# uni-medical/UniMedVL

Hardware: AMD Instinct MI355X
Metric: VQA greedy decode tokens/s, UniMedVL-14B (BAGEL-7B-MoT dims), batch 8 x 448x448 per GPU (higher is better)
Workload: dtype bf16; 1 GPU; configs[1]: UniMedVL-14B bf16 VQA greedy decode, batch=8 448x448, 1xMI355X; batch_per_gpu=8, image=448x448, parallelism=dp1, decode=hipGraph

## Files before the change

### include/unimedvl_hip.h

```cpp
#ifndef UNIMEDVL_HIP_H
#define UNIMEDVL_HIP_H
#include <stddef.h>
#include <stdint.h>

#ifdef __cplusplus
extern "C" {
#endif

typedef void* umv_stream_t;

int umv_version(void);
const char* umv_last_error(void);

size_t umv_packed_weight_elems(int N, int K);
int umv_pack_weight_bf16(const uint16_t* w, uint16_t* packed, int N, int K, umv_stream_t stream);
size_t umv_repacked_weight_elems(int N, int K, int th);
int umv_repack_weight_rows_bf16(const uint16_t* packed16, uint16_t* out, int N, int K, int th, umv_stream_t stream);
int umv_pack_weight_swiglu_bf16(const uint16_t* gate, const uint16_t* up, uint16_t* packed, int I, int K,
                                umv_stream_t stream);

enum {
    UMV_EPI_BIAS = 1,
    UMV_EPI_GELU_TANH = 2,
    UMV_EPI_SILU = 4,
    UMV_EPI_RESIDUAL = 8,
    UMV_EPI_SWIGLU = 16,
    UMV_EPI_OUT_F32 = 32
};
typedef struct {
    uint64_t seed;
    int64_t  draw;
    uint32_t stream;
    float    temperature;
    int32_t  top_k;
    float    top_p;
    float    min_p;
    float    repetition_penalty, presence_penalty, frequency_penalty;
} umv_row_sampling;
typedef struct {
    const uint16_t* x;
    int64_t ldx;
    const uint16_t* wp;
    const uint16_t* bias;
    const uint16_t* residual;
    int64_t ldr;
    void* out;
    int64_t ldo;
    const int32_t* row_idx;
    int M, N, K;
    int epilogue;
    const uint16_t* norm_w;
    float norm_eps;
    int tile_rows;
    const float* w_scale;
    int k_splits;
    int64_t split_stride;
    uint64_t* argmax_partial;
    int64_t x_rows;
    float sample_temperature;
    uint64_t sample_seed;
    const int64_t* sample_step;
    float* lse_partial;
} umv_gemm_args;
int umv_gemm_bf16(const umv_gemm_args* a, umv_stream_t stream);
int umv_gemm_bf16_rows(const umv_gemm_args* a, const umv_row_sampling* rows, umv_stream_t stream);
int umv_gemm_tile_config(int M, int N, int K);

size_t umv_packed_weight_fp8_bytes(int N, int K);
int umv_quantize_pack_weight_fp8(const uint16_t* w, const uint16_t* w_up, uint8_t* packed8, float* scale, uint16_t* deq,
                                 uint16_t* deq_up, int rows, int K, umv_stream_t stream);
int umv_gemm_fp8w(const umv_gemm_args* a, umv_stream_t stream);
int umv_gemm_fp8w_rows(const umv_gemm_args* a, const umv_row_sampling* rows, umv_stream_t stream);

size_t umv_packed_weight_mxfp4_bytes(int N, int K);
int umv_quantize_pack_weight_mxfp4(const uint16_t* w, const uint16_t* w_up, uint8_t* packed4, uint16_t* deq, uint16_t* deq_up,
                                   int rows, int K, umv_stream_t stream);
int umv_gemm_mxfp4w(const umv_gemm_args* a, umv_stream_t stream);
int umv_gemm_mxfp4t(const umv_gemm_args* a, umv_stream_t stream);

size_t umv_packed_weight_z13_bytes(int N, int K);
int umv_pack_weight_z13(const uint16_t* packed16, uint8_t* z13, int N, int K, umv_stream_t stream);
int umv_gemm_z13w(const umv_gemm_args* a, const void* z13, umv_stream_t stream);
int umv_gemm_z13w_rows(const umv_gemm_args* a, const void* z13, const umv_row_sampling* rows, umv_stream_t stream);

size_t umv_packed_weight_fp8_mfma_bytes(int N, int K);
int umv_repack_weight_fp8_mfma(const uint8_t* packed8, uint8_t* out, int N, int K, umv_stream_t stream);
int umv_quantize_act_fp8(const uint16_t* x, int64_t ldx, const int32_t* row_idx, uint8_t* xq, int64_t ldq, float* x_scale,
                         uint16_t* deq, int64_t ldd, int M, int K, umv_stream_t stream);
typedef struct {
    const uint8_t* xq;
    int64_t ldq;
    const float* x_scale;
    const uint8_t* wp;
    const float* w_scale;
    const uint16_t* bias;
    const uint16_t* residual;
    int64_t ldr;
    void* out;
    int64_t ldo;
    const int32_t* row_idx;
    int M, N, K;
    int epilogue;
} umv_gemm8_args;
int umv_gemm_fp8a8w(const umv_gemm8_args* a, umv_stream_t stream);

int umv_rmsnorm_bf16(const uint16_t* x, const uint16_t* w, const uint16_t* w_gen, const int32_t* expert,
                     uint16_t* out, int T, int H, float eps, umv_stream_t stream);
int umv_residual_rmsnorm_bf16(const float* partials, int n_splits, int64_t split_stride, int64_t ldp, uint16_t* seq,
                              const uint16_t* w, uint16_t* out, int T, int H, float eps, umv_stream_t stream);
int umv_layernorm_bf16(const uint16_t* x, const uint16_t* w, const uint16_t* b, uint16_t* out, int T, int H,
                       float eps, umv_stream_t stream);
int umv_embed_gather_bf16(const uint16_t* table, const int64_t* ids, const int32_t* out_rows, uint16_t* out,
                          int T, int H, umv_stream_t stream);
int umv_add_rows_bf16(const uint16_t* a, const uint16_t* bcast, const uint16_t* table, const int64_t* idx,
                      const int32_t* out_rows, uint16_t* out, int T, int H, umv_stream_t stream);
int umv_argmax_bf16(const uint16_t* logits, int64_t ld, int64_t* out_ids, int M, int V, umv_stream_t stream);
int umv_sample_bf16(const uint16_t* logits, int64_t ld, int64_t* out_ids, int M, int V, float temperature, uint64_t seed,
                    const int64_t* step, umv_stream_t stream);
int umv_cast_pad_f32_bf16(const float* x, int64_t ldx, uint16_t* out, int64_t ldo, int T, int K, int Kp,
                          umv_stream_t stream);
int umv_patchify_f32_bf16(const float* img, int C, int H, int W, int p, uint16_t* out, int64_t ldo, int Kp, umv_stream_t stream);


typedef struct {
    const uint16_t* qkv;
    uint16_t* q_out;
    uint16_t* k_slab;
    uint16_t* vt_slab;
    int64_t k_seg_stride, k_head_stride, v_seg_stride, v_head_stride, v_d_stride;
    const int32_t *tok_seg, *tok_slot, *tok_pos, *expert;
    const uint16_t *q_norm_w, *k_norm_w, *q_norm_w_gen, *k_norm_w_gen;
    const uint16_t *cos_tab, *sin_tab;
    int T, nq, nkv, hd;
    float eps;
    int fp32_chain;
    const float* qkv_partials;
    int n_splits;
    int64_t split_stride;
    const uint16_t* qkv_bias;
    const int32_t* page_table;
    int page_table_stride;
} umv_qkv_post_args;
int umv_qkv_post(const umv_qkv_post_args* a, umv_stream_t stream);

typedef struct {
    const uint16_t* q;
    uint16_t* out;
    const int32_t* cu_q;
    const int32_t* kv_len;
    const uint16_t* k_slab;
    const uint16_t* vt_slab;
    int64_t k_seg_stride, k_head_stride, v_seg_stride, v_head_stride, v_d_stride;
    int nseg, nq, nkv, hd, causal;
    int max_q;
    int max_kv;
    int nsplit;
    void* workspace;
    int64_t q_row_stride, k_key_stride;
    int variant;
    uint32_t* stats;
    const int32_t* page_table;
    int page_table_stride;
    int wave_split;
} umv_attn_args;
#define UMV_KV_PAGE 256
#define UMV_KV_PAGE_LOG2 8
// ... 127 lines not shown
```

### unimedvl_amd/_lib.py

```python
import ctypes as C
import os

HERE = os.path.dirname(os.path.abspath(__file__))
LIB_PATH = os.environ.get("UMV_LIB_PATH") or os.path.join(HERE, "lib", "libunimedvl_hip.so")

EPI_BIAS, EPI_GELU_TANH, EPI_SILU, EPI_RESIDUAL, EPI_SWIGLU, EPI_OUT_F32 = 1, 2, 4, 8, 16, 32


class GemmArgs(C.Structure):
    _fields_ = [
        ("x", C.c_void_p), ("ldx", C.c_int64), ("wp", C.c_void_p), ("bias", C.c_void_p),
        ("residual", C.c_void_p), ("ldr", C.c_int64), ("out", C.c_void_p), ("ldo", C.c_int64),
        ("row_idx", C.c_void_p), ("M", C.c_int), ("N", C.c_int), ("K", C.c_int), ("epilogue", C.c_int),
        ("norm_w", C.c_void_p), ("norm_eps", C.c_float), ("tile_rows", C.c_int), ("w_scale", C.c_void_p),
        ("k_splits", C.c_int), ("split_stride", C.c_int64), ("argmax_partial", C.c_void_p), ("x_rows", C.c_int64),
        ("sample_temperature", C.c_float), ("sample_seed", C.c_uint64), ("sample_step", C.c_void_p),
        ("lse_partial", C.c_void_p),
    ]


class QkvPostArgs(C.Structure):
    _fields_ = [
        ("qkv", C.c_void_p), ("q_out", C.c_void_p), ("k_slab", C.c_void_p), ("vt_slab", C.c_void_p),
        ("k_seg_stride", C.c_int64), ("k_head_stride", C.c_int64), ("v_seg_stride", C.c_int64),
# ... 16 lines not shown
        ("v_head_stride", C.c_int64), ("v_d_stride", C.c_int64),
        ("nseg", C.c_int), ("nq", C.c_int), ("nkv", C.c_int), ("hd", C.c_int), ("causal", C.c_int),
        ("max_q", C.c_int), ("max_kv", C.c_int), ("nsplit", C.c_int), ("workspace", C.c_void_p),
        ("q_row_stride", C.c_int64), ("k_key_stride", C.c_int64),
        ("variant", C.c_int), ("stats", C.c_void_p),
        ("page_table", C.c_void_p), ("page_table_stride", C.c_int), ("wave_split", C.c_int),
    ]


ATTN_FORCE, ATTN_STREAM, ATTN_TQ1, ATTN_TQ2, ATTN_EXACT, ATTN_WHOLE_TOKENS = 1, 2, 4, 8, 16, 32
ATTN_PAIR = 64


class Gemm8Args(C.Structure):
    _fields_ = [
        ("xq", C.c_void_p), ("ldq", C.c_int64), ("x_scale", C.c_void_p), ("wp", C.c_void_p), ("w_scale", C.c_void_p),
        ("bias", C.c_void_p), ("residual", C.c_void_p), ("ldr", C.c_int64), ("out", C.c_void_p), ("ldo", C.c_int64),
        ("row_idx", C.c_void_p), ("M", C.c_int), ("N", C.c_int), ("K", C.c_int), ("epilogue", C.c_int),
    ]


class LogitPenaltyArgs(C.Structure):
    _fields_ = [
        ("logits", C.c_void_p), ("ld", C.c_int64), ("ids", C.c_void_p), ("count", C.c_void_p), ("list", C.c_void_p),
        ("list_len", C.c_void_p), ("bias", C.c_void_p), ("M", C.c_int), ("V", C.c_int), ("cap", C.c_int), ("n_static", C.c_int),
        ("repetition_penalty", C.c_float), ("presence_penalty", C.c_float), ("frequency_penalty", C.c_float),
        ("temperature", C.c_float), ("argmax_partial", C.c_void_p), ("lse_partial", C.c_void_p), ("n_tiles", C.c_int),
        ("seed", C.c_uint64), ("step", C.c_void_p), ("rows", C.c_void_p),
    ]


class RowSampling(C.Structure):
    _fields_ = [
        ("seed", C.c_uint64), ("draw", C.c_int64), ("stream", C.c_uint32), ("temperature", C.c_float), ("top_k", C.c_int32),
        ("top_p", C.c_float), ("min_p", C.c_float), ("repetition_penalty", C.c_float), ("presence_penalty", C.c_float),
        ("frequency_penalty", C.c_float),
    ]


class SpecStepArgs(C.Structure):
    _fields_ = [
        ("tok_slot", C.c_void_p), ("tok_pos", C.c_void_p), ("kv_len", C.c_void_p), ("argmax_partial", C.c_void_p),
        ("n_tiles", C.c_int), ("V", C.c_int), ("ids", C.c_void_p), ("out_ids", C.c_void_p), ("out_ld", C.c_int64),
        ("n_out", C.c_void_p), ("limit", C.c_void_p), ("n_draft", C.c_void_p), ("hist", C.c_void_p), ("hist_ld", C.c_int64),
        ("hist_len", C.c_void_p), ("predicted", C.c_void_p), ("pred_ld", C.c_int64), ("pred_len", C.c_void_p), ("stats", C.c_void_p),
        ("B", C.c_int), ("k", C.c_int), ("ngram_min", C.c_int), ("ngram_max", C.c_int), ("draft_only", C.c_int),
    ]


PENALTY_COUNT_MASK, PENALTY_CONTEXT, PENALTY_LISTED = 0x3FFFFFFF, 0x40000000, 0x80000000
TOP_LOGPROBS_MAX, TOP_AFTER_LOGPROB, TOP_AFTER_TRUNCATED = 20, 0, 1


_SIGS = {
    "umv_packed_weight_fp8_mfma_bytes": (C.c_size_t, [C.c_int, C.c_int]),
    "umv_repack_weight_fp8_mfma": (C.c_int, [C.c_void_p, C.c_void_p, C.c_int, C.c_int, C.c_void_p]),
    "umv_quantize_act_fp8": (C.c_int, [C.c_void_p, C.c_int64, C.c_void_p, C.c_void_p, C.c_int64, C.c_void_p, C.c_void_p, C.c_int64,
                                       C.c_int, C.c_int, C.c_void_p]),
    "umv_gemm_fp8a8w": (C.c_int, [C.POINTER(Gemm8Args), C.c_void_p]),
    "umv_gemm_tile_config": (C.c_int, [C.c_int, C.c_int, C.c_int]),
    "umv_attn_prefill_tq": (C.c_int, [C.c_int, C.c_int, C.c_int, C.c_int, C.c_int]),
    "umv_version": (C.c_int, []),
    "umv_last_error": (C.c_char_p, []),
    "umv_packed_weight_elems": (C.c_size_t, [C.c_int, C.c_int]),
    "umv_pack_weight_bf16": (C.c_int, [C.c_void_p, C.c_void_p, C.c_int, C.c_int, C.c_void_p]),
    "umv_repacked_weight_elems": (C.c_size_t, [C.c_int, C.c_int, C.c_int]),
    "umv_repack_weight_rows_bf16": (C.c_int, [C.c_void_p, C.c_void_p, C.c_int, C.c_int, C.c_int, C.c_void_p]),
    "umv_pack_weight_swiglu_bf16": (C.c_int, [C.c_void_p, C.c_void_p, C.c_void_p, C.c_int, C.c_int, C.c_void_p]),
    "umv_gemm_bf16": (C.c_int, [C.POINTER(GemmArgs), C.c_void_p]),
    "umv_packed_weight_fp8_bytes": (C.c_size_t, [C.c_int, C.c_int]),
    "umv_quantize_pack_weight_fp8": (C.c_int, [C.c_void_p, C.c_void_p, C.c_void_p, C.c_void_p, C.c_void_p, C.c_void_p,
                                               C.c_int, C.c_int, C.c_void_p]),
    "umv_gemm_fp8w": (C.c_int, [C.POINTER(GemmArgs), C.c_void_p]),
    "umv_gemm_bf16_rows": (C.c_int, [C.POINTER(GemmArgs), C.c_void_p, C.c_void_p]),
    "umv_gemm_fp8w_rows": (C.c_int, [C.POINTER(GemmArgs), C.c_void_p, C.c_void_p]),
    "umv_gemm_z13w_rows": (C.c_int, [C.POINTER(GemmArgs), C.c_void_p, C.c_void_p, C.c_void_p]),
    "umv_packed_weight_mxfp4_bytes": (C.c_size_t, [C.c_int, C.c_int]),
    "umv_quantize_pack_weight_mxfp4": (C.c_int, [C.c_void_p, C.c_void_p, C.c_void_p, C.c_void_p, C.c_void_p, C.c_int, C.c_int,
                                                 C.c_void_p]),
    "umv_gemm_mxfp4w": (C.c_int, [C.POINTER(GemmArgs), C.c_void_p]),
    "umv_packed_weight_z13_bytes": (C.c_size_t, [C.c_int, C.c_int]),
    "umv_pack_weight_z13": (C.c_int, [C.c_void_p, C.c_void_p, C.c_int, C.c_int, C.c_void_p]),
    "umv_gemm_z13w": (C.c_int, [C.POINTER(GemmArgs), C.c_void_p, C.c_void_p]),
    "umv_gemm_mxfp4t": (C.c_int, [C.POINTER(GemmArgs), C.c_void_p]),
    "umv_residual_rmsnorm_bf16": (C.c_int, [C.c_void_p, C.c_int, C.c_int64, C.c_int64, C.c_void_p, C.c_void_p, C.c_void_p, C.c_int,
                                            C.c_int, C.c_float, C.c_void_p]),
    "umv_rmsnorm_bf16": (C.c_int, [C.c_void_p, C.c_void_p, C.c_void_p, C.c_void_p, C.c_void_p, C.c_int, C.c_int,
                                   C.c_float, C.c_void_p]),
    "umv_layernorm_bf16": (C.c_int, [C.c_void_p, C.c_void_p, C.c_void_p, C.c_void_p, C.c_int, C.c_int, C.c_float,
                                     C.c_void_p]),
    "umv_embed_gather_bf16": (C.c_int, [C.c_void_p, C.c_void_p, C.c_void_p, C.c_void_p, C.c_int, C.c_int, C.c_void_p]),
    "umv_add_rows_bf16": (C.c_int, [C.c_void_p, C.c_void_p, C.c_void_p, C.c_void_p, C.c_void_p, C.c_void_p, C.c_int,
                                    C.c_int, C.c_void_p]),
    "umv_argmax_bf16": (C.c_int, [C.c_void_p, C.c_int64, C.c_void_p, C.c_int, C.c_int, C.c_void_p]),
    "umv_sample_bf16": (C.c_int, [C.c_void_p, C.c_int64, C.c_void_p, C.c_int, C.c_int, C.c_float, C.c_uint64, C.c_void_p,
                                  C.c_void_p]),
    "umv_cast_pad_f32_bf16": (C.c_int, [C.c_void_p, C.c_int64, C.c_void_p, C.c_int64, C.c_int, C.c_int, C.c_int,
                                        C.c_void_p]),
    "umv_patchify_f32_bf16": (C.c_int, [C.c_void_p, C.c_int, C.c_int, C.c_int, C.c_int, C.c_void_p, C.c_int64, C.c_int, C.c_void_p]),
    "umv_qkv_post": (C.c_int, [C.POINTER(QkvPostArgs), C.c_void_p]),
    "umv_attn_workspace_bytes": (C.c_size_t, [C.c_int, C.c_int, C.c_int, C.c_int, C.c_int]),
    "umv_attn_varlen": (C.c_int, [C.POINTER(AttnArgs), C.c_void_p]),
    "umv_decode_advance": (C.c_int, [C.c_void_p, C.c_void_p, C.c_void_p, C.c_int, C.c_void_p]),
    "umv_decode_step_end": (C.c_int, [C.c_void_p, C.c_void_p, C.c_void_p, C.c_void_p, C.c_void_p, C.c_void_p, C.c_void_p, C.c_int,
                                      C.c_int, C.c_void_p]),
    "umv_decode_step_end_argmax": (C.c_int, [C.c_void_p, C.c_void_p, C.c_void_p, C.c_void_p, C.c_int, C.c_void_p, C.c_void_p, C.c_void_p,
                                             C.c_void_p, C.c_int, C.c_int, C.c_void_p]),
    "umv_decode_step_end_logprob": (C.c_int, [C.c_void_p, C.c_void_p, C.c_void_p, C.c_void_p, C.c_void_p, C.c_int, C.c_void_p, C.c_void_p,
                                              C.c_void_p, C.c_void_p, C.c_void_p, C.c_int64, C.c_int, C.c_float, C.c_void_p, C.c_void_p,
                                              C.c_int, C.c_int, C.c_void_p]),
    "umv_token_logprob_bf16": (C.c_int, [C.c_void_p, C.c_int64, C.c_void_p, C.c_void_p, C.c_int, C.c_int, C.c_float, C.c_void_p]),
    "umv_sample_truncated_bf16": (C.c_int, [C.c_void_p, C.c_int64, C.c_void_p, C.c_int, C.c_int, C.c_float, C.c_uint64, C.c_void_p,
                                            C.c_int, C.c_float, C.c_float, C.c_void_p, C.c_void_p, C.c_void_p]),
    "umv_decode_step_end_truncated": (C.c_int, [C.c_void_p, C.c_void_p, C.c_void_p, C.c_void_p, C.c_void_p, C.c_int, C.c_void_p, C.c_void_p,
                                                C.c_void_p, C.c_void_p, C.c_void_p, C.c_int64, C.c_int, C.c_float, C.c_void_p, C.c_void_p,
                                                C.c_int, C.c_int, C.c_uint64, C.c_int, C.c_float, C.c_float, C.c_void_p, C.c_void_p,
                                                C.c_void_p]),
    "umv_decode_step_end_rows": (C.c_int, [C.c_void_p, C.c_void_p, C.c_void_p, C.c_void_p, C.c_void_p, C.c_int, C.c_void_p, C.c_void_p,
                                           C.c_void_p, C.c_void_p, C.c_void_p, C.c_int64, C.c_int, C.c_void_p, C.c_void_p, C.c_int, C.c_int,
                                           C.c_void_p, C.c_void_p, C.c_void_p, C.c_void_p]),
    "umv_decode_top_logprobs": (C.c_int, [C.c_void_p, C.c_int64, C.c_int, C.c_void_p, C.c_int, C.c_float, C.c_void_p, C.c_int, C.c_void_p,
                                          C.c_void_p, C.c_void_p, C.c_int, C.c_int, C.c_int, C.c_void_p, C.c_void_p, C.c_void_p, C.c_void_p]),
    "umv_top_logprobs_bf16": (C.c_int, [C.c_void_p, C.c_int64, C.c_void_p, C.c_int, C.c_int, C.c_float, C.c_int, C.c_void_p, C.c_void_p,
                                        C.c_void_p, C.c_void_p]),
    "umv_logit_penalty_bf16": (C.c_int, [C.POINTER(LogitPenaltyArgs), C.c_void_p]),
    "umv_decode_step_end_speculative": (C.c_int, [C.POINTER(SpecStepArgs), C.c_void_p]),
    "umv_timestep_embed": (C.c_int, [C.c_void_p, C.c_void_p, C.c_void_p, C.c_int, C.c_int, C.c_void_p]),
    "umv_cfg_renorm_euler": (C.c_int, [C.c_void_p, C.c_void_p, C.c_void_p, C.c_void_p, C.c_int64, C.c_void_p, C.c_void_p,
                                       C.c_int, C.c_float, C.c_float, C.c_float, C.c_int, C.c_float, C.c_int, C.c_void_p]),
    "umv_conv2d_nhwc_bf16": (C.c_int, [C.c_void_p, C.c_void_p, C.c_void_p, C.c_void_p, C.c_void_p, C.c_int, C.c_int,
                                       C.c_int, C.c_int, C.c_int, C.c_int, C.c_int, C.c_void_p]),
    "umv_groupnorm_workspace_bytes": (C.c_size_t, [C.c_int, C.c_int]),
    "umv_groupnorm_nhwc_bf16": (C.c_int, [C.c_void_p, C.c_void_p, C.c_void_p, C.c_void_p, C.c_void_p, C.c_int, C.c_int,
                                          C.c_int, C.c_float, C.c_int, C.c_void_p]),
    "umv_nchw_f32_to_nhwc_bf16": (C.c_int, [C.c_void_p, C.c_void_p, C.c_int, C.c_int, C.c_int, C.c_int, C.c_int,
                                            C.c_void_p]),
    "umv_unpatchify_latent": (C.c_int, [C.c_void_p, C.c_void_p, C.c_int, C.c_int, C.c_int, C.c_int, C.c_float,
                                        C.c_float, C.c_void_p]),
    "umv_pixels_to_u8": (C.c_int, [C.c_void_p, C.c_void_p, C.c_int64, C.c_int, C.c_void_p]),
    "umv_softmax_rows_f32": (C.c_int, [C.c_void_p, C.c_int64, C.c_void_p, C.c_int64, C.c_void_p, C.c_int, C.c_int, C.c_float, C.c_void_p]),
    "umv_rowscale_f32_bf16": (C.c_int, [C.c_void_p, C.c_int64, C.c_void_p, C.c_void_p, C.c_int64, C.c_int, C.c_int, C.c_void_p]),
    "umv_latent_sample_patchify": (C.c_int, [C.c_void_p, C.c_void_p, C.c_void_p, C.c_int, C.c_int, C.c_int, C.c_int,
                                             C.c_int, C.c_int, C.c_int, C.c_float, C.c_float, C.c_void_p]),
}

_lib = None


class UmvError(RuntimeError):
    pass


def load():
    global _lib
    if _lib is not None:
        return _lib
    import torch
    if not os.path.exists(LIB_PATH):
        raise UmvError(
            f"{LIB_PATH} not found: build it with `python -m unimedvl_amd.build` "
            "(there is no CPU or PyTorch fallback for the product path)")
    lib = C.CDLL(LIB_PATH)
    for name, (res, args) in _SIGS.items():
        fn = getattr(lib, name)
        fn.restype = res
        fn.argtypes = args
# ... 13 lines not shown
```

### unimedvl_amd/csrc/gemm_z13.hip

```cpp
#include "common.h"
#include "../../include/unimedvl_hip.h"
#include "gemm_skinny.h"

#define UMV_SKINNY13_KERNEL(NAME, ROWS, ROWS_ARG, ROWS_USE)                                                                                                 \
    template <int MB, int NP, int U, int XL = 0>                                                                                        \
    __global__ __launch_bounds__(SK_WAVES * 64) void NAME(umv_gemm_args a, const uint8_t* z13, int KT8, int NTT, int NPT ROWS_ARG) {   \
                                                           \
        const int KT = 2 * KT8, nsplit = a.k_splits > 1 ? a.k_splits : 1;                                                               \
        const int kts = (KT + nsplit - 1) / nsplit;                                                                                     \
        const int ks0 = (int)blockIdx.y * kts, ks1 = min(KT, ks0 + kts);                                                                \
        uint64_t any = 0;                                                                                                               \
        if (ks1 > ks0) {                                                                                                                \
            const int b0 = ks0 >> 4, b1 = (ks1 + 15) >> 4;                                                 \
            const uint64_t range = (b1 - b0 >= 64 ? ~0ull : ((1ull << (b1 - b0)) - 1ull)) << b0;                                        \
            const uint64_t* flags = reinterpret_cast<const uint64_t*>(z13);                                                             \
            _Pragma("unroll") for (int i = 0; i < NP; ++i) {                                                                            \
                const int p = (int)blockIdx.x * NP + i;                                                                                 \
                if (p < NPT) any |= flags[2 * p] & range;               \
            }                                                                                                                           \
        }                                                                                                                               \
        if (any != 0) {                                                                                                                 \
            gemm_skinny_body<SkBf16<2 * NP>, MB, 2 * U, true, 0, XL, ROWS>(a, KT, NTT, 0 ROWS_USE);                                     \
        } else {                                                                                                                        \
            a.wp = reinterpret_cast<const uint16_t*>(z13);                                                                              \
            gemm_skinny_body<SkZ13<NP>, MB, U, true, 0, XL, ROWS>(a, KT8, NTT, NPT ROWS_USE);                                           \
        }                                                                                                                               \
    }
#define UMV_COMMA ,
UMV_SKINNY13_KERNEL(gemm_skinny13_kernel, false, , )
UMV_SKINNY13_KERNEL(gemm_skinny13_rows_kernel, true, UMV_COMMA const umv_row_sampling* rows, UMV_COMMA rows)
#undef UMV_COMMA
#undef UMV_SKINNY13_KERNEL

template <int MB, int NP, int U>
static int launch_skinny13(const umv_gemm_args& a, const uint8_t* z13, int KT8, int NTT, int NPT, hipStream_t s) {
    return launch_skinny_body<MB, 2 * NP, U, 2, 0>([](auto XL) { return &gemm_skinny13_kernel<MB, NP, U, decltype(XL)::value>; }, a, KT8,
                                                   NTT, s, z13, KT8, NTT, NPT);
}
template <int MB, int NP, int U>
static int launch_skinny13_rows(const umv_gemm_args& a, const uint8_t* z13, int KT8, int NTT, int NPT, hipStream_t s,
                                const umv_row_sampling* rows) {
    return launch_skinny_body<MB, 2 * NP, U, 2, 0>([](auto XL) { return &gemm_skinny13_rows_kernel<MB, NP, U, decltype(XL)::value>; }, a, KT8,
                                                   NTT, s, z13, KT8, NTT, NPT, rows);
}

static int gemm_z13w(const umv_gemm_args* ap, const void* z13, const umv_row_sampling* rows, umv_stream_t stream) {
    UMV_CHECK(ap != nullptr, UMV_ERR_ARG, "gemm_z13w: null args");
    umv_gemm_args a = *ap;
    UMV_CHECK(a.x && a.wp && a.out && z13, UMV_ERR_ARG, "gemm_z13w: null pointer (x, wp = the bf16 image, out and z13 are required)");
    UMV_CHECK(!a.w_scale, UMV_ERR_ARG, "gemm_z13w: w_scale must be NULL");
    if (const int rc = umv_gemm_check_args(a, "gemm_z13w", 32)) return rc;
    UMV_CHECK((a.K % 64) == 0 && a.K <= 32768, UMV_ERR_UNSUPPORTED, "gemm_z13w: K (%d) must be a multiple of 64 and <= 32768", a.K);
    if (const int rc = umv_gemm_check_decode(a, "gemm_z13w", "13-bit", "umv_gemm_bf16", true, true)) return rc;
    UMV_CHECK(((uintptr_t)z13 % 256) == 0, UMV_ERR_ARG, "gemm_z13w: the 13-bit image must be 256-byte aligned");
    if (a.M == 0) return UMV_OK;
    hipStream_t s = (hipStream_t)stream;
    const uint8_t* z = reinterpret_cast<const uint8_t*>(z13);
    const int KT8 = a.K / 64, NTT = (a.N + 15) / 16, NPT = (NTT + 1) / 2;
    if (a.k_splits > 1) {
        if (a.M <= 16) return launch_skinny13<1, 2, 1>(a, z, KT8, NTT, NPT, s);
        if (a.M <= 32) return launch_skinny13<2, 2, 1>(a, z, KT8, NTT, NPT, s);
        return launch_skinny13<4, 1, 1>(a, z, KT8, NTT, NPT, s);
    }
    const bool two = (a.epilogue & UMV_EPI_SWIGLU) || NTT >= 1024;
    if (rows) {
        if (a.M <= 16) return launch_skinny13_rows<1, 1, 2>(a, z, KT8, NTT, NPT, s, rows);
        if (a.M <= 32)
            return two ? launch_skinny13_rows<2, 2, 1>(a, z, KT8, NTT, NPT, s, rows) : launch_skinny13_rows<2, 1, 2>(a, z, KT8, NTT, NPT, s, rows);
        return launch_skinny13_rows<4, 1, 1>(a, z, KT8, NTT, NPT, s, rows);
    }
    if (a.M <= 16) return launch_skinny13<1, 1, 2>(a, z, KT8, NTT, NPT, s);
    if (a.M <= 32) return two ? launch_skinny13<2, 2, 1>(a, z, KT8, NTT, NPT, s) : launch_skinny13<2, 1, 2>(a, z, KT8, NTT, NPT, s);
    if (two && !a.argmax_partial && a.K >= 1024) return umv_gemm_bf16(&a, stream);
    return launch_skinny13<4, 1, 1>(a, z, KT8, NTT, NPT, s);
}

extern "C" int umv_gemm_z13w(const umv_gemm_args* ap, const void* z13, umv_stream_t stream) { return gemm_z13w(ap, z13, nullptr, stream); }
extern "C" int umv_gemm_z13w_rows(const umv_gemm_args* ap, const void* z13, const umv_row_sampling* rows, umv_stream_t stream) {
    UMV_CHECK(ap != nullptr, UMV_ERR_ARG, "gemm_z13w_rows: null args");
    if (const int rc = umv_gemm_check_rows(*ap, rows, "gemm_z13w_rows")) return rc;
    return gemm_z13w(ap, z13, rows, stream);
}
```

### unimedvl_amd/ops.py

```python
import ctypes as C
import functools

import torch

from . import _lib
from ._lib import (EPI_BIAS, EPI_GELU_TANH, EPI_OUT_F32, EPI_RESIDUAL, EPI_SILU, EPI_SWIGLU, AttnArgs, GemmArgs,
                   LogitPenaltyArgs, QkvPostArgs, check)

BF16 = torch.bfloat16


_raw_stream = getattr(torch._C, "_cuda_getCurrentRawStream", None)


def _stream():
    if _raw_stream is not None:
        return C.c_void_p(_raw_stream(torch.cuda.current_device()))
    return C.c_void_p(torch.cuda.current_stream().cuda_stream)


def on_device(fn):
    @functools.wraps(fn)
    def wrapper(self, *args, **kwargs):
        dev = torch.device(self.device)
        if dev.type != "cuda" or dev.index is None or dev.index == torch.cuda.current_device():
            return fn(self, *args, **kwargs)
        with torch.cuda.device(dev):
            return fn(self, *args, **kwargs)
    return wrapper


def device_scope(device):
    dev = torch.device(device)
    if dev.type != "cuda" or dev.index is None:
        import contextlib
        return contextlib.nullcontext()
    return torch.cuda.device(dev)


def _p(t):
    return None if t is None else C.c_void_p(t.data_ptr())


def _req(t, dtype, name):
    if not t.is_cuda:
        raise _lib.UmvError(f"{name}: tensor must live on the GPU (no CPU fallback)")
    if t.dtype != dtype:
        raise _lib.UmvError(f"{name}: expected {dtype}, got {t.dtype}")
    return t


Z13_MAX_ROWS = 32


class PackedLinear:

    __slots__ = ("wp", "bias", "N", "K", "swiglu", "th", "w8", "scale", "w8m", "w4", "wz")

    def __init__(self, wp, bias, N, K, swiglu=False, th=16, w8=None, scale=None, w4=None):
        self.wp, self.bias, self.N, self.K, self.swiglu, self.th = wp, bias, N, K, swiglu, th
        self.w8, self.scale = w8, scale
        self.w8m = None
        self.w4 = w4
        self.wz = None

    def build_z13(self):
        if self.wp is None or self.th != 16 or self.w8 is not None or self.w4 is not None or self.K % 64 or self.K > 32768:
            raise _lib.UmvError("build_z13 needs a plain bf16 linear (16-row image) with K a multiple of 64, K <= 32768")
        lib = _lib.load()
        self.wz = torch.empty(lib.umv_packed_weight_z13_bytes(self.N, self.K), dtype=torch.uint8, device=self.wp.device)
        check(lib.umv_pack_weight_z13(_p(self.wp), _p(self.wz), self.N, self.K, _stream()), "umv_pack_weight_z13")
        return self

    def drop_bf16(self):
        if self.w4 is None:
            raise _lib.UmvError("drop_bf16 needs MXFP4 weights (from_weight_mxfp4 / from_gate_up_mxfp4)")
        self.wp = None
        return self

    def enable_fp8_mfma(self, keep_bf16=False):
        if self.w8m is not None:
            if not keep_bf16:
                self.wp = None
            return self
        if self.w8 is None:
            raise _lib.UmvError("enable_fp8_mfma needs fp8 weights (from_weight_fp8 / from_gate_up_fp8)")
        lib = _lib.load()
        self.w8m = torch.empty(lib.umv_packed_weight_fp8_mfma_bytes(self.N, self.K), dtype=torch.uint8, device=self.w8.device)
        check(lib.umv_repack_weight_fp8_mfma(_p(self.w8), _p(self.w8m), self.N, self.K, _stream()), "umv_repack_weight_fp8_mfma")
        if not keep_bf16:
            self.wp = None
        return self

    @staticmethod
    def _operands(w, up):
        if up is None:
            w = _req(w.contiguous(), BF16, "weight")
        else:
            w, up = _req(w.contiguous(), BF16, "gate"), _req(up.contiguous(), BF16, "up")
            assert w.shape[0] % 16 == 0, "intermediate size must be a multiple of 16"
        rows, K = w.shape
        return w, up, rows, rows if up is None else 2 * rows, K

    @staticmethod
    def _bf16(w, up=None, bias=None):
        lib = _lib.load()
        w, up, rows, N, K = PackedLinear._operands(w, up)
        wp = torch.empty(lib.umv_packed_weight_elems(N, K), dtype=BF16, device=w.device)
        if up is None:
            check(lib.umv_pack_weight_bf16(_p(w), _p(wp), N, K, _stream()), "umv_pack_weight_bf16")
        else:
            check(lib.umv_pack_weight_swiglu_bf16(_p(w), _p(up), _p(wp), rows, K, _stream()), "umv_pack_weight_swiglu_bf16")
        return PackedLinear(wp, None if bias is None else bias.contiguous(), N, K, swiglu=up is not None)

    @staticmethod
    def _quantized(fmt, w, up=None, bias=None, keep_bf16=True):
        lib = _lib.load()
        w, up, rows, N, K = PackedLinear._operands(w, up)
        img = torch.empty(getattr(lib, f"umv_packed_weight_{fmt}_bytes")(N, K), dtype=torch.uint8, device=w.device)
        scale = torch.empty((N + 15) // 16 * 16, dtype=torch.float32, device=w.device) if fmt == "fp8" else None
        deq = torch.empty_like(w) if keep_bf16 else None
        deq_up = torch.empty_like(up) if keep_bf16 and up is not None else None
        images = (_p(img), _p(scale)) if fmt == "fp8" else (_p(img),)
        check(getattr(lib, f"umv_quantize_pack_weight_{fmt}")(_p(w), _p(up), *images, _p(deq), _p(deq_up), rows, K, _stream()),
              f"umv_quantize_pack_weight_{fmt}")
        if keep_bf16:
            lin = PackedLinear._bf16(deq, deq_up, bias)
        else:
            lin = PackedLinear(None, None if bias is None else bias.contiguous(), N, K, swiglu=up is not None)
        if fmt == "fp8":
            lin.w8, lin.scale = img, scale
        else:
            lin.w4 = img
        return lin

    @staticmethod
    def from_weight_fp8(w, bias=None):
        return PackedLinear._quantized("fp8", w, None, bias)

    @staticmethod
    def from_gate_up_fp8(gate, up):
        return PackedLinear._quantized("fp8", gate, up)

    @staticmethod
    def from_weight_mxfp4(w, bias=None, keep_bf16=True):
        return PackedLinear._quantized("mxfp4", w, None, bias, keep_bf16)

    @staticmethod
    def from_gate_up_mxfp4(gate, up, keep_bf16=True):
        return PackedLinear._quantized("mxfp4", gate, up, None, keep_bf16)

    @staticmethod
    def from_weight(w, bias=None):
        return PackedLinear._bf16(w, None, bias)

    @staticmethod
    def from_gate_up(gate, up):
        return PackedLinear._bf16(gate, up)

    def for_decode(self, n_cus=256):
        if self.swiglu or self.th != 16 or self.w8 is not None or self.w4 is not None:
            return self
        best = None
        for th in range(15, 7, -1):
            if self.N % th == 0 and (self.N // th) % n_cus == 0:
                best = th
                break
        if best is None or ((self.N + 15) // 16) % n_cus == 0:
            return self
        lib = _lib.load()
        out = torch.empty(lib.umv_repacked_weight_elems(self.N, self.K, best), dtype=BF16, device=self.wp.device)
        check(lib.umv_repack_weight_rows_bf16(_p(self.wp), _p(out), self.N, self.K, best, _stream()), "umv_repack_weight_rows_bf16")
        return PackedLinear(out, self.bias, self.N, self.K, False, best)

    def nbytes(self):
        return self.wp.numel() * 2 if self.wp is not None else self.w4.numel()

    def decode_bytes(self):
        for image in (self.w8, self.w4, self.wz):
            if image is not None:
                return image.numel()
        return self.wp.numel() * 2


def _z13_takes(lin, M, z13, form):
    if lin.wz is None or z13 is False:
        return False
    if z13:
        return M <= 64
    if form == "splitk":
        return M <= Z13_MAX_ROWS
    return form == "epilogue" and (M <= 8 or 16 < M <= Z13_MAX_ROWS)


def _route(lin, M, splitk=False, norm=False, amax=False, act8=False, out_f32=False, act=False, z13=None):
    if act8 and lin.w8m is None:
        raise _lib.UmvError("act8 needs a linear with the fp8-MFMA image (enable_fp8_mfma)")
    skinny = M <= 64 and not norm
    if act8 and not splitk and M > 64 and not norm and not out_f32:
        return "umv_gemm_fp8a8w", lin.w8m, lin.scale, None
    if lin.w8 is not None and (skinny or splitk):
        return "umv_gemm_fp8w", lin.w8, lin.scale, None
    if lin.w4 is not None:
        if skinny:
            return "umv_gemm_mxfp4w", lin.w4, None, None
        if lin.wp is None:
            if not splitk and (norm or amax):
                raise _lib.UmvError(f"this linear only has its fp4 (MXFP4) image (built with keep_bf16=False / drop_bf16): M={M} rows with "
                                    f"norm_w={'set' if norm else 'None'}, argmax_partial={'set' if amax else 'None'} need "
                                    "the bf16 kernel - build the weights with keep_bf16=True (llm_fp4_keep_bf16=True)")
            return "umv_gemm_mxfp4t", lin.w4, None, None
    if lin.wp is None and not splitk:
        raise _lib.UmvError(f"this linear only has fp8 images (the bf16 image was dropped by enable_fp8_mfma): M={M} rows with "
                            f"act8={act8}, out_f32={out_f32}, norm_w={'set' if norm else 'None'} need the bf16 kernel - "
                            "build the weights with enable_fp8_mfma(keep_bf16=True)")
    if _z13_takes(lin, M, z13, "splitk" if splitk else "epilogue" if (lin.swiglu or amax) else None) and not norm and not act:
        return "umv_gemm_z13w", lin.wp, None, lin.wz
    return "umv_gemm_bf16", lin.wp, None, None


def _launch(lib, route, x, lin, out, ldo, M, flags=0, residual=None, row_idx=None, norm_w=None, norm_eps=0.0, amax=None, sample=None,
            k_splits=0, split_stride=0, lse=None, sample_rows=None):
    entry, image, scale, wz = route
    a = GemmArgs(x=x.data_ptr(), ldx=x.stride(0), wp=None if image is None else image.data_ptr(), out=out.data_ptr(), ldo=ldo,
                 M=M, N=lin.N, K=lin.K, epilogue=flags, norm_eps=norm_eps, argmax_partial=amax)
    if flags & EPI_BIAS:
        a.bias = lin.bias.data_ptr()
    if residual is not None:
        a.residual, a.ldr = residual.data_ptr(), residual.stride(0)
    if row_idx is not None:
        a.row_idx = row_idx.data_ptr()
    if norm_w is not None:
        a.norm_w = norm_w.data_ptr()
    if scale is not None:
        a.w_scale = scale.data_ptr()
    if k_splits:
        a.k_splits, a.split_stride = k_splits, split_stride
    elif entry in ("umv_gemm_bf16", "umv_gemm_z13w"):
        a.tile_rows, a.x_rows = lin.th, x.shape[0]
    if sample is not None and entry not in ("umv_gemm_mxfp4w", "umv_gemm_mxfp4t"):
        a.sample_temperature, a.sample_seed, a.sample_step = _sample_fields(sample, amax)
    if lse is not None:
        a.lse_partial = lse
    if sample_rows is not None:
        if wz is not None:
            check(lib.umv_gemm_z13w_rows(C.byref(a), wz.data_ptr(), sample_rows, _stream()), entry + "_rows")
        else:
            check(getattr(lib, entry + "_rows")(C.byref(a), sample_rows, _stream()), entry + "_rows")
    elif wz is not None:
        check(lib.umv_gemm_z13w(C.byref(a), wz.data_ptr(), _stream()), entry)
    else:
        check(getattr(lib, entry)(C.byref(a), _stream()), entry)
    return out


def gemm(x, lin, out=None, *, M=None, residual=None, act=None, row_idx=None, out_f32=False, use_bias=True,
         norm_w=None, norm_eps=1e-6, act8=False, argmax_partial=None, sample=None, z13=None, lse_partial=None, sample_rows=None):
    lib = _lib.load()
    _req(x, BF16, "x")
    assert x.stride(-1) == 1
    M = x.shape[0] if M is None else M
    flags = 0
    if lin.bias is not None and use_bias:
        flags |= EPI_BIAS
    if act == "gelu_tanh":
        flags |= EPI_GELU_TANH
    elif act == "silu":
        flags |= EPI_SILU
    elif act is not None:
        raise ValueError(act)
    if lin.swiglu:
        flags |= EPI_SWIGLU
    if residual is not None:
        flags |= EPI_RESIDUAL
    if out_f32:
        flags |= EPI_OUT_F32
    if out is None:
        assert row_idx is None, "row-indexed GEMM writes into a caller-provided buffer"
        out = torch.empty((x.shape[0], lin.N // 2 if lin.swiglu else lin.N), dtype=torch.float32 if out_f32 else BF16, device=x.device)
    route = _route(lin, M, False, norm_w is not None, argmax_partial is not None, act8, out_f32, act is not None, z13)
    if act8 and M <= 64:
        x = fake_quantize_act(x, M, row_idx)
    amax = None
    if argmax_partial is not None:
        _req(argmax_partial, torch.int64, "argmax_partial")
        if not (argmax_partial.is_contiguous() and tuple(argmax_partial.shape) == (M, (lin.N + 15) // 16)):
            raise _lib.UmvError(f"argmax_partial must be a contiguous int64 [{M}, {(lin.N + 15) // 16}] tensor")
        amax = argmax_partial.data_ptr()
    lse = None
    if lse_partial is not None:
        _req(lse_partial, torch.float32, "lse_partial")
        if not (lse_partial.is_contiguous() and tuple(lse_partial.shape) == (M, (lin.N + 15) // 16, 2)):
            raise _lib.UmvError(f"lse_partial must be a contiguous fp32 [{M}, {(lin.N + 15) // 16}, 2] tensor")
        lse = lse_partial.data_ptr()
    rows = None
    if sample_rows is not None:
        if route[0] not in ("umv_gemm_bf16", "umv_gemm_z13w", "umv_gemm_fp8w"):
            raise _lib.UmvError(f"gemm: sample_rows rides on the argmax_partial epilogue of the bf16 / 13-bit / e4m3 routes, not {route[0]}")
        rows = _row_table(sample_rows, M, "gemm")
    if route[0] == "umv_gemm_fp8a8w":
        if lse is not None:
            raise _lib.UmvError("gemm: lse_partial rides on the argmax_partial epilogue of the M <= 64 kernels")
        xq, xs = quantize_act(x, M, row_idx, lin.K)
        a8 = _lib.Gemm8Args(xq=xq.data_ptr(), ldq=xq.stride(0), x_scale=xs.data_ptr(), wp=lin.w8m.data_ptr(), w_scale=lin.scale.data_ptr(),
                            out=out.data_ptr(), ldo=out.stride(0), M=M, N=lin.N, K=lin.K, epilogue=flags)
        if flags & EPI_BIAS:
            a8.bias = lin.bias.data_ptr()
        if residual is not None:
            a8.residual, a8.ldr = residual.data_ptr(), residual.stride(0)
        if row_idx is not None:
            a8.row_idx = row_idx.data_ptr()
        check(lib.umv_gemm_fp8a8w(C.byref(a8), _stream()), "umv_gemm_fp8a8w")
        return out
    return _launch(lib, route, x, lin, out, out.stride(0), M, flags, residual, row_idx, norm_w, norm_eps, amax, sample, lse=lse,
                   sample_rows=rows)


def rmsnorm(x, w, eps, out=None, w_gen=None, expert=None):
    lib = _lib.load()
    _req(x, BF16, "x")
    T, H = x.shape
    out = torch.empty_like(x) if out is None else out
    check(lib.umv_rmsnorm_bf16(_p(x), _p(w), _p(w_gen), _p(expert), _p(out), T, H, eps, _stream()), "umv_rmsnorm_bf16")
    return out


def layernorm(x, w, b, eps, out=None):
    lib = _lib.load()
    _req(x, BF16, "x")
    T, H = x.shape
    out = torch.empty_like(x) if out is None else out
    check(lib.umv_layernorm_bf16(_p(x), _p(w), _p(b), _p(out), T, H, eps, _stream()), "umv_layernorm_bf16")
    return out
# ... 558 lines not shown
```

Baseline: 2692 tokens/s.

## Pass host-side z13 escape-flag bitmap to skip per-tile bf16 fallback checks

Keeps a host copy of the per-pair escape flag words from the head of the 13-bit weight image. At launch it builds a per-workgroup bitmap passed as a kernel argument, so each workgroup knows up front whether its tile needs the bf16 fallback path or can run the pure z13 path. This removes per-tile runtime flag reads and divergent fallback handling from the skinny decode GEMMs. The cost is extra host work per launch to build the map (baked in under hipGraph capture) and a larger kernel argument block; the flag copy must stay in sync with the device image, and an optional environment check verifies this.

```diff
diff --git a/include/unimedvl_hip.h b/include/unimedvl_hip.h
--- a/include/unimedvl_hip.h
+++ b/include/unimedvl_hip.h
@@ -82,6 +82,10 @@
 int umv_pack_weight_z13(const uint16_t* packed16, uint8_t* z13, int N, int K, umv_stream_t stream);
 int umv_gemm_z13w(const umv_gemm_args* a, const void* z13, umv_stream_t stream);
 int umv_gemm_z13w_rows(const umv_gemm_args* a, const void* z13, const umv_row_sampling* rows, umv_stream_t stream);
+int umv_gemm_z13w_hf(const umv_gemm_args* a, const void* z13, const uint64_t* host_flags, umv_stream_t stream);
+int umv_gemm_z13w_rows_hf(const umv_gemm_args* a, const void* z13, const uint64_t* host_flags, const umv_row_sampling* rows,
+                          umv_stream_t stream);
+int umv_gemm_z13w_flag_map(const uint64_t* host_flags, int NP, int pairs_per_wg, int grid_x, int k_splits, int K, uint32_t* map);
 
 size_t umv_packed_weight_fp8_mfma_bytes(int N, int K);
 int umv_repack_weight_fp8_mfma(const uint8_t* packed8, uint8_t* out, int N, int K, umv_stream_t stream);
diff --git a/unimedvl_amd/_lib.py b/unimedvl_amd/_lib.py
--- a/unimedvl_amd/_lib.py
+++ b/unimedvl_amd/_lib.py
@@ -122,6 +122,9 @@
     "umv_packed_weight_z13_bytes": (C.c_size_t, [C.c_int, C.c_int]),
     "umv_pack_weight_z13": (C.c_int, [C.c_void_p, C.c_void_p, C.c_int, C.c_int, C.c_void_p]),
     "umv_gemm_z13w": (C.c_int, [C.POINTER(GemmArgs), C.c_void_p, C.c_void_p]),
+    "umv_gemm_z13w_hf": (C.c_int, [C.POINTER(GemmArgs), C.c_void_p, C.c_void_p, C.c_void_p]),
+    "umv_gemm_z13w_rows_hf": (C.c_int, [C.POINTER(GemmArgs), C.c_void_p, C.c_void_p, C.c_void_p, C.c_void_p]),
+    "umv_gemm_z13w_flag_map": (C.c_int, [C.c_void_p, C.c_int, C.c_int, C.c_int, C.c_int, C.c_int, C.c_void_p]),
     "umv_gemm_mxfp4t": (C.c_int, [C.POINTER(GemmArgs), C.c_void_p]),
     "umv_residual_rmsnorm_bf16": (C.c_int, [C.c_void_p, C.c_int, C.c_int64, C.c_int64, C.c_void_p, C.c_void_p, C.c_void_p, C.c_int,
                                             C.c_int, C.c_float, C.c_void_p]),
diff --git a/unimedvl_amd/csrc/gemm_z13.hip b/unimedvl_amd/csrc/gemm_z13.hip
--- a/unimedvl_amd/csrc/gemm_z13.hip
+++ b/unimedvl_amd/csrc/gemm_z13.hip
@@ -29,8 +29,57 @@
 #define UMV_COMMA ,
 UMV_SKINNY13_KERNEL(gemm_skinny13_kernel, false, , )
 UMV_SKINNY13_KERNEL(gemm_skinny13_rows_kernel, true, UMV_COMMA const umv_row_sampling* rows, UMV_COMMA rows)
+#undef UMV_SKINNY13_KERNEL
+
+#define UMV_Z13_MAP_WORDS 160
+struct umv_z13_map { uint32_t w[UMV_Z13_MAP_WORDS]; };
+#define UMV_SKINNY13M_KERNEL(NAME, ROWS, ROWS_ARG, ROWS_USE)                                                                            \
+    template <int MB, int NP, int U, int XL = 0>                                                                                        \
+    __global__ __launch_bounds__(SK_WAVES * 64) void NAME(umv_gemm_args a, const uint8_t* z13, int KT8, int NTT, int NPT ROWS_ARG,      \
+                                                          const umv_z13_map map) {                                                      \
+         \
+                                                                                                                    \
+        const int wg = NP == 1 ? (int)blockIdx.x : (int)blockIdx.y * ((NPT + NP - 1) / NP) + (int)blockIdx.x;                           \
+        const uint32_t any = (map.w[wg >> 5] >> (wg & 31)) & 1u;                                                                        \
+        if (any != 0) {                                                                                                                 \
+            gemm_skinny_body<SkBf16<2 * NP>, MB, 2 * U, true, 0, XL, ROWS>(a, 2 * KT8, NTT, 0 ROWS_USE);                                \
+        } else {                                                                                                                        \
+            a.wp = reinterpret_cast<const uint16_t*>(z13);                                                                              \
+            gemm_skinny_body<SkZ13<NP>, MB, U, true, 0, XL, ROWS>(a, KT8, NTT, NPT ROWS_USE);                                           \
+        }                                                                                                                               \
+    }
+UMV_SKINNY13M_KERNEL(gemm_skinny13m_kernel, false, , )
+UMV_SKINNY13M_KERNEL(gemm_skinny13m_rows_kernel, true, UMV_COMMA const umv_row_sampling* rows, UMV_COMMA rows)
 #undef UMV_COMMA
-#undef UMV_SKINNY13_KERNEL
+#undef UMV_SKINNY13M_KERNEL
+
+static bool z13_build_map(const uint64_t* flags, int NPT, int NP, int gx, int gy, int K, uint32_t* w) {
+    if (gx < 1 || gy < 1 || (long long)gx * gy > 32ll * UMV_Z13_MAP_WORDS) return false;
+    for (int i = 0; i < UMV_Z13_MAP_WORDS; ++i) w[i] = 0;
+    const int KT = K / 32, kts = (KT + gy - 1) / gy;
+    for (int y = 0; y < gy; ++y) {
+        const int ks0 = y * kts, ks1 = ks0 + kts < KT ? ks0 + kts : KT;
+        if (ks1 <= ks0) continue;
+        const int b0 = ks0 >> 4, b1 = (ks1 + 15) >> 4;
+        const uint64_t range = (b1 - b0 >= 64 ? ~0ull : ((1ull << (b1 - b0)) - 1ull)) << b0;
+        for (int x = 0; x < gx; ++x) {
+            uint64_t any = 0;
+            for (int i = 0; i < NP; ++i) {
+                const int p = x * NP + i;
+                if (p < NPT) any |= flags[p] & range;
+            }
+            const int bit = y * gx + x;
+            if (any) w[bit >> 5] |= 1u << (bit & 31);
+        }
+    }
+    return true;
+}
+
+extern "C" int umv_gemm_z13w_flag_map(const uint64_t* host_flags, int NPT, int pairs_per_wg, int grid_x, int k_splits, int K,
+                                      uint32_t* map) {
+    if (!host_flags || !map || NPT < 1 || pairs_per_wg < 1 || K < 64 || (K % 64) != 0 || K > 32768) return -1;
+    return z13_build_map(host_flags, NPT, pairs_per_wg, grid_x, k_splits > 1 ? k_splits : 1, K, map) ? 1 : 0;
+}
 
 template <int MB, int NP, int U>
 static int launch_skinny13(const umv_gemm_args& a, const uint8_t* z13, int KT8, int NTT, int NPT, hipStream_t s) {
@@ -44,7 +93,25 @@
                                                    NTT, s, z13, KT8, NTT, NPT, rows);
 }
 
-static int gemm_z13w(const umv_gemm_args* ap, const void* z13, const umv_row_sampling* rows, umv_stream_t stream) {
+template <int MB, int NP, int U>
+static int launch_skinny13m(const umv_gemm_args& a, const uint8_t* z13, int KT8, int NTT, int NPT, hipStream_t s, const uint64_t* hf) {
+    umv_z13_map map;
+    if (!hf || (NP == 1 && a.k_splits > 1) || !z13_build_map(hf, NPT, NP, (NTT + 2 * NP - 1) / (2 * NP), a.k_splits > 1 ? a.k_splits : 1, a.K, map.w))
+        return launch_skinny13<MB, NP, U>(a, z13, KT8, NTT, NPT, s);
+    return launch_skinny_body<MB, 2 * NP, U, 2, 0>([](auto XL) { return &gemm_skinny13m_kernel<MB, NP, U, decltype(XL)::value>; }, a, KT8,
+                                                   NTT, s, z13, KT8, NTT, NPT, map);
+}
+template <int MB, int NP, int U>
+static int launch_skinny13m_rows(const umv_gemm_args& a, const uint8_t* z13, int KT8, int NTT, int NPT, hipStream_t s,
+                                 const umv_row_sampling* rows, const uint64_t* hf) {
+    umv_z13_map map;
+    if (!hf || (NP == 1 && a.k_splits > 1) || !z13_build_map(hf, NPT, NP, (NTT + 2 * NP - 1) / (2 * NP), a.k_splits > 1 ? a.k_splits : 1, a.K, map.w))
+        return launch_skinny13_rows<MB, NP, U>(a, z13, KT8, NTT, NPT, s, rows);
+    return launch_skinny_body<MB, 2 * NP, U, 2, 0>([](auto XL) { return &gemm_skinny13m_rows_kernel<MB, NP, U, decltype(XL)::value>; }, a,
+                                                   KT8, NTT, s, z13, KT8, NTT, NPT, rows, map);
+}
+
+static int gemm_z13w(const umv_gemm_args* ap, const void* z13, const umv_row_sampling* rows, const uint64_t* hf, umv_stream_t stream) {
     UMV_CHECK(ap != nullptr, UMV_ERR_ARG, "gemm_z13w: null args");
     umv_gemm_args a = *ap;
     UMV_CHECK(a.x && a.wp && a.out && z13, UMV_ERR_ARG, "gemm_z13w: null pointer (x, wp = the bf16 image, out and z13 are required)");
@@ -58,26 +125,35 @@
     const uint8_t* z = reinterpret_cast<const uint8_t*>(z13);
     const int KT8 = a.K / 64, NTT = (a.N + 15) / 16, NPT = (NTT + 1) / 2;
     if (a.k_splits > 1) {
-        if (a.M <= 16) return launch_skinny13<1, 2, 1>(a, z, KT8, NTT, NPT, s);
-        if (a.M <= 32) return launch_skinny13<2, 2, 1>(a, z, KT8, NTT, NPT, s);
+        if (a.M <= 16) return launch_skinny13m<1, 2, 1>(a, z, KT8, NTT, NPT, s, hf);
+        if (a.M <= 32) return launch_skinny13m<2, 2, 1>(a, z, KT8, NTT, NPT, s, hf);
         return launch_skinny13<4, 1, 1>(a, z, KT8, NTT, NPT, s);
     }
     const bool two = (a.epilogue & UMV_EPI_SWIGLU) || NTT >= 1024;
     if (rows) {
-        if (a.M <= 16) return launch_skinny13_rows<1, 1, 2>(a, z, KT8, NTT, NPT, s, rows);
+        if (a.M <= 16) return launch_skinny13m_rows<1, 1, 2>(a, z, KT8, NTT, NPT, s, rows, hf);
         if (a.M <= 32)
-            return two ? launch_skinny13_rows<2, 2, 1>(a, z, KT8, NTT, NPT, s, rows) : launch_skinny13_rows<2, 1, 2>(a, z, KT8, NTT, NPT, s, rows);
+            return two ? launch_skinny13m_rows<2, 2, 1>(a, z, KT8, NTT, NPT, s, rows, hf) : launch_skinny13_rows<2, 1, 2>(a, z, KT8, NTT, NPT, s, rows);
         return launch_skinny13_rows<4, 1, 1>(a, z, KT8, NTT, NPT, s, rows);
     }
-    if (a.M <= 16) return launch_skinny13<1, 1, 2>(a, z, KT8, NTT, NPT, s);
-    if (a.M <= 32) return two ? launch_skinny13<2, 2, 1>(a, z, KT8, NTT, NPT, s) : launch_skinny13<2, 1, 2>(a, z, KT8, NTT, NPT, s);
+    if (a.M <= 16) return launch_skinny13m<1, 1, 2>(a, z, KT8, NTT, NPT, s, hf);
+    if (a.M <= 32) return two ? launch_skinny13m<2, 2, 1>(a, z, KT8, NTT, NPT, s, hf) : launch_skinny13m<2, 1, 2>(a, z, KT8, NTT, NPT, s, hf);
     if (two && !a.argmax_partial && a.K >= 1024) return umv_gemm_bf16(&a, stream);
     return launch_skinny13<4, 1, 1>(a, z, KT8, NTT, NPT, s);
 }
 
-extern "C" int umv_gemm_z13w(const umv_gemm_args* ap, const void* z13, umv_stream_t stream) { return gemm_z13w(ap, z13, nullptr, stream); }
+extern "C" int umv_gemm_z13w(const umv_gemm_args* ap, const void* z13, umv_stream_t stream) { return gemm_z13w(ap, z13, nullptr, nullptr, stream); }
 extern "C" int umv_gemm_z13w_rows(const umv_gemm_args* ap, const void* z13, const umv_row_sampling* rows, umv_stream_t stream) {
     UMV_CHECK(ap != nullptr, UMV_ERR_ARG, "gemm_z13w_rows: null args");
     if (const int rc = umv_gemm_check_rows(*ap, rows, "gemm_z13w_rows")) return rc;
-    return gemm_z13w(ap, z13, rows, stream);
+    return gemm_z13w(ap, z13, rows, nullptr, stream);
 }
+extern "C" int umv_gemm_z13w_hf(const umv_gemm_args* ap, const void* z13, const uint64_t* host_flags, umv_stream_t stream) {
+    return gemm_z13w(ap, z13, nullptr, host_flags, stream);
+}
+extern "C" int umv_gemm_z13w_rows_hf(const umv_gemm_args* ap, const void* z13, const uint64_t* host_flags, const umv_row_sampling* rows,
+                                     umv_stream_t stream) {
+    UMV_CHECK(ap != nullptr, UMV_ERR_ARG, "gemm_z13w_rows: null args");
+    if (const int rc = umv_gemm_check_rows(*ap, rows, "gemm_z13w_rows")) return rc;
+    return gemm_z13w(ap, z13, rows, host_flags, stream);
+}
diff --git a/unimedvl_amd/ops.py b/unimedvl_amd/ops.py
--- a/unimedvl_amd/ops.py
+++ b/unimedvl_amd/ops.py
@@ -1,5 +1,6 @@
 import ctypes as C
 import functools
+import os
 
 import torch
 
@@ -55,7 +56,7 @@
 
 class PackedLinear:
 
-    __slots__ = ("wp", "bias", "N", "K", "swiglu", "th", "w8", "scale", "w8m", "w4", "wz")
+    __slots__ = ("wp", "bias", "N", "K", "swiglu", "th", "w8", "scale", "w8m", "w4", "wz", "wz_flags")
 
     def __init__(self, wp, bias, N, K, swiglu=False, th=16, w8=None, scale=None, w4=None):
         self.wp, self.bias, self.N, self.K, self.swiglu, self.th = wp, bias, N, K, swiglu, th
@@ -63,6 +64,7 @@
         self.w8m = None
         self.w4 = w4
         self.wz = None
+        self.wz_flags = None
 
     def build_z13(self):
         if self.wp is None or self.th != 16 or self.w8 is not None or self.w4 is not None or self.K % 64 or self.K > 32768:
@@ -70,6 +72,8 @@
         lib = _lib.load()
         self.wz = torch.empty(lib.umv_packed_weight_z13_bytes(self.N, self.K), dtype=torch.uint8, device=self.wp.device)
         check(lib.umv_pack_weight_z13(_p(self.wp), _p(self.wz), self.N, self.K, _stream()), "umv_pack_weight_z13")
+        pairs = ((self.N + 15) // 16 + 1) // 2
+        self.wz_flags = self.wz[:16 * pairs].cpu().view(torch.int64)[0::2].contiguous()
         return self
 
     def drop_bf16(self):
@@ -217,6 +221,20 @@
     if _z13_takes(lin, M, z13, "splitk" if splitk else "epilogue" if (lin.swiglu or amax) else None) and not norm and not act:
         return "umv_gemm_z13w", lin.wp, None, lin.wz
     return "umv_gemm_bf16", lin.wp, None, None
+
+
+Z13_FLAGMAP = True
+
+
+def _z13_host_flags(lin, wz):
+    hf = lin.wz_flags if wz is lin.wz else None
+    env = os.environ.get("UMV_Z13_FLAGMAP", "")
+    if hf is None or (env == "0" if env else not Z13_FLAGMAP):
+        return None
+    if os.environ.get("UMV_Z13_FLAGMAP_CHECK", "0") == "1" and not (wz.is_cuda and torch.cuda.is_current_stream_capturing()):
+        if hf.numel() * 16 > wz.numel() or not torch.equal(wz[:16 * hf.numel()].cpu().view(torch.int64)[0::2], hf):
+            raise _lib.UmvError("umv_gemm_z13w_hf: the host copy of the flag words differs from the head of the 13-bit image")
+    return hf
 
 
 def _launch(lib, route, x, lin, out, ldo, M, flags=0, residual=None, row_idx=None, norm_w=None, norm_eps=0.0, amax=None, sample=None,
@@ -244,11 +262,19 @@
         a.lse_partial = lse
     if sample_rows is not None:
         if wz is not None:
-            check(lib.umv_gemm_z13w_rows(C.byref(a), wz.data_ptr(), sample_rows, _stream()), entry + "_rows")
+            hf = _z13_host_flags(lin, wz)
+            if hf is not None:
+                check(lib.umv_gemm_z13w_rows_hf(C.byref(a), wz.data_ptr(), hf.data_ptr(), sample_rows, _stream()), entry + "_rows_hf")
+            else:
+                check(lib.umv_gemm_z13w_rows(C.byref(a), wz.data_ptr(), sample_rows, _stream()), entry + "_rows")
         else:
             check(getattr(lib, entry + "_rows")(C.byref(a), sample_rows, _stream()), entry + "_rows")
     elif wz is not None:
-        check(lib.umv_gemm_z13w(C.byref(a), wz.data_ptr(), _stream()), entry)
+        hf = _z13_host_flags(lin, wz)
+        if hf is not None:
+            check(lib.umv_gemm_z13w_hf(C.byref(a), wz.data_ptr(), hf.data_ptr(), _stream()), entry + "_hf")
+        else:
+            check(lib.umv_gemm_z13w(C.byref(a), wz.data_ptr(), _stream()), entry)
     else:
         check(getattr(lib, entry)(C.byref(a), _stream()), entry)
     return out
```

Measured after the change: 2712 tokens/s, median of 6. No clear change (+0.8%).
